# JuliaReinforcementLearning/ReinforcementLearning.jl

Measured on NVIDIA H100. Metric: env-steps/sec at 65536 CartPole envs (full PPO iteration: rollout T=32 + GAE + 4 epochs x 4 minibatches), higher is better.
Workload: dtype f32

## Files before the change

### reinforcementlearning.jl_b200/csrc/nn_tc.cu

```cuda
#include "nn.cuh"
#include "perm.cuh"
#include "policy.cuh"
#include "tc_fwd.cuh"
#include "tc_split.h"
#include "wgmma.cuh"

namespace {

using tcfwd::G_F;
using tcfwd::GW_S;
using tcfwd::WIMG_BYTES;
using tcfwd::split2;
using tcfwd::wimg_off;
constexpr int TM = tcfwd::TM;
constexpr int H = tcfwd::H;
constexpr float kScaleW = tcfwd::kScale;

constexpr int NT7 = 512;
constexpr int kMaxStage = 10;
constexpr int GF_T = 128;
constexpr int GS_T = 16 * GF_T;
constexpr int FIMG = 8 * GS_T;
constexpr float kScaleH = 64.0f, kScaleX = 64.0f;
constexpr int kNo = 2;

struct SmemBwd {
    static_assert(FIMG % 128 == 0 && WIMG_BYTES % 128 == 0 && (2 * GS_T) % 16 == 0, "operand images must stay 128-byte aligned");
    alignas(128) uint8_t FP_full[FIMG];
    alignas(128) uint8_t FP_lo[FIMG];
    alignas(128) uint8_t FH_lo[FIMG];
    alignas(128) uint8_t FH_full[FIMG];
    alignas(128) uint8_t FQ_full[FIMG];
    alignas(128) uint8_t FQ_lo[FIMG];
    alignas(128) uint8_t B1[WIMG_BYTES];
    alignas(128) uint8_t XT[2][2 * GS_T];
    alignas(128) uint8_t AH_full[FIMG];
    alignas(128) uint8_t AH_lo[FIMG];
    alignas(16) float D[TM * H];
    uint64_t H1pos[2][TM];
    float W1[kInMax * H];
    float b1[H], b2[H];
    float W3[H * kNo];
    float b3[kNo];
    float Zp[4 * kNo * TM];
    float Red[32];
    double RedD[16];
    float step_scale;
    alignas(8) uint64_t bar1;
    alignas(8) uint64_t bar3;
    alignas(8) uint64_t bar4;
    float AccW2[64 * 65 + 64];
    float AccD4[64 * 9];
};
__device__ __forceinline__ int d_off(int s, int col) { return s * H + ((((col >> 2) ^ (s & 15))) << 2) + (col & 3); }
__device__ __forceinline__ void d_ld16(const float* D, int s, int f0, float (&v)[16]) {
#pragma unroll
    for (int u = 0; u < 4; ++u) {
        const float4 q4 = *reinterpret_cast<const float4*>(D + d_off(s, f0 + 4 * u));
        v[4 * u] = q4.x; v[4 * u + 1] = q4.y; v[4 * u + 2] = q4.z; v[4 * u + 3] = q4.w;
    }
}
template <int TB>
__device__ __forceinline__ void gemm_ts3(float (&d)[32], const uint8_t* a_hi, const uint8_t* a_lo, int h, uint64_t dB, uint32_t b_step) {
    const uint64_t dA = wg::make_desc(wg::smem_u32(a_hi) + 8 * h * GF_T, GS_T, GF_T), dAl = wg::make_desc(wg::smem_u32(a_lo) + 8 * h * GF_T, GS_T, GF_T);
    wg::fence();
#pragma unroll
    for (int k = 0; k < 4; ++k) {
        const uint32_t aa = k * 2 * GS_T, bb = k * b_step;
        wg::mma_m64n64k16<0, TB>(d, wg::desc_add(dA, aa), wg::desc_add(dB, bb), k ? 1u : 0u);
        wg::mma_m64n64k16<0, TB>(d, wg::desc_add(dA, aa), wg::desc_add(dB, 8 * GW_S + bb), 1u);
        wg::mma_m64n64k16<0, TB>(d, wg::desc_add(dAl, aa), wg::desc_add(dB, bb), 1u);
    }
    wg::commit();
    wg::wait_all();
}
__device__ __forceinline__ uint32_t fimg_off(int f, int s) { return (uint32_t)((f >> 3) * GS_T + (s >> 3) * GF_T + (s & 7) * 16 + (f & 7) * 2); }
__device__ __forceinline__ void store16_feat(uint8_t* img, int f0, int s, const uint32_t (&v)[8]) {
    uint8_t* p = img + fimg_off(f0, s);
    *reinterpret_cast<uint4*>(p) = make_uint4(v[0], v[1], v[2], v[3]);
    *reinterpret_cast<uint4*>(p + GS_T) = make_uint4(v[4], v[5], v[6], v[7]);
}
using b200perm::perm_index;
using b200perm::perm_index_bits;

__device__ __forceinline__ float lane_transpose_reduce32(float (&v)[32], int lane) {
#pragma unroll
    for (int st = 0; st < 5; ++st) {
        const int half = 16 >> st, off = 16 >> st;
        const bool upper = (lane & off) != 0;
#pragma unroll
        for (int n = 0; n < half; ++n) {
            float send = upper ? v[n] : v[n + half];
            float keep = upper ? v[n + half] : v[n];
            v[n] = keep + __shfl_xor_sync(0xffffffffu, send, off);
        }
    }
    return v[0];
}

__device__ __forceinline__ void worker_sync() { asm volatile("bar.sync 1, 512;" ::: "memory"); }
__device__ __forceinline__ void group_sync(int q) { asm volatile("bar.sync %0, 128;" ::"r"(5 + q) : "memory"); }
__device__ __forceinline__ void ready_arrive(int id) { asm volatile("bar.arrive %0, 640;" ::"r"(id) : "memory"); }
__device__ __forceinline__ void ready_wait(int id) { asm volatile("bar.sync %0, 640;" ::"r"(id) : "memory"); }
#ifdef B200RL_K7_TIMING
__device__ unsigned long long g_k7_phase[40];
__device__ int g_k7_watch = 0;
#define K7_T(i) do { if (tid == (g_k7_watch & 0xFFFF) && (int)blockIdx.x == (g_k7_watch >> 16)) { long long now_ = clock64(); g_k7_phase[i] += (unsigned long long)(now_ - tprev_); tprev_ = now_; } } while (0)
#else
#define K7_T(i) do { } while (0)
#endif
constexpr int NT7_ALL = NT7 + 128;
constexpr int kRegsMma = 64, kRegsWorker = 104;
static_assert(128 * kRegsMma + NT7 * kRegsWorker <= NT7_ALL * 96, "setmaxnreg split must fit the CTA's register allocation");
constexpr int kBarRdyA = 2, kBarRdyB = 3;
constexpr int kBarMma = 4;
__device__ __forceinline__ void mma_sync() { asm volatile("bar.sync %0, 128;" ::"n"(kBarMma) : "memory"); }

template <int ACT>
__global__ void __launch_bounds__(NT7_ALL, 1)
ac_loss_grad_tc_kernel(MlpDesc actor, MlpDesc critic, const float* params , AcHyper hp, AcBatch b, float* partial,
                       float* __restrict__ loss_partial, int64_t np_total, float scale_base ,
                       OptStep st ,
                       int n_actor ) {
    extern __shared__ __align__(1024) unsigned char smem_raw[];
    SmemBwd& sm = *reinterpret_cast<SmemBwd*>(smem_raw);
    const int role = (int)blockIdx.x < n_actor ? 0 : 1;
    const int cta = role ? (int)blockIdx.x - n_actor : (int)blockIdx.x;
    const int nctas = role ? (int)gridDim.x - n_actor : n_actor;
    const int nrows = max(n_actor, (int)gridDim.x - n_actor);
    const float scale_p = scale_base * (role ? 4.0f : 64.0f);
    const MlpDesc d = role ? critic : actor;
    const int act = ACT >= 0 ? ACT : d.act;
    const bool relu = act == B200RL_ACT_RELU;
    const int64_t poff = role ? actor.nparams() : 0;
    const float* __restrict__ p = params + poff;
    const int tid = threadIdx.x, warp = tid >> 5, lane = tid & 31;
    const int q = warp & 3, c = (warp >> 2) & 3;
    const int s = 32 * q + lane;
    {
        const float* b1 = p + (int64_t)H * d.in;
        const float* W2 = b1 + H;
        const float* b2 = W2 + (int64_t)H * H;
        const float s1 = relu ? kScaleH : 1.0f;
        for (int k = tid; k < kInMax * H; k += NT7_ALL) sm.W1[k] = (k / H) < d.in ? p[k] * s1 : 0.f;
        for (int k = tid; k < H; k += NT7_ALL) { sm.b1[k] = b1[k] * s1; sm.b2[k] = b2[k]; }
        for (int k = tid; k < H * kNo; k += NT7_ALL) {
            int j = k / kNo, o = k % kNo;
            sm.W3[k] = o < d.nout ? p[head_w<false>(d, o, j)] : 0.f;
        }
        if (tid < kNo) sm.b3[tid] = tid < d.nout ? p[head_b<false>(d, tid)] : 0.f;
        tcfwd::fill_w2_image<NT7_ALL>(sm.B1, W2);
    }
    if (tid == 32) {
        wg::mbar_init(&sm.bar1, 128); wg::mbar_init(&sm.bar3, 128); wg::mbar_init(&sm.bar4, 128);
    }
    wg::fence_proxy_async();
    __syncthreads();
    const float inv_s1 = 1.0f / (kScaleH * kScaleW), inv_s3 = 1.0f / (scale_p * kScaleH), inv_sp = 1.0f / scale_p, inv_s4 = 1.0f / (scale_p * kScaleX);
    const int64_t ntiles = (b.B + TM - 1) / TM;

    if (warp >= NT7 / 32) {
        asm volatile("setmaxnreg.dec.sync.aligned.u32 %0;" ::"n"(kRegsMma));
        const int t = tid - NT7, row0 = 16 * (t >> 5) + ((t & 31) >> 2), col0 = 2 * (t & 3);
        const uint64_t dB1k = wg::make_desc(wg::smem_u32(sm.B1), G_F, GW_S);
        const uint64_t dB1t = wg::make_desc(wg::smem_u32(sm.B1), GW_S, G_F);
        float dacc[32];
        auto store_d = [&](int h) {
#pragma unroll
            for (int j = 0; j < 8; ++j)
#pragma unroll
                for (int hh = 0; hh < 2; ++hh)
                    *reinterpret_cast<float2*>(sm.D + d_off(64 * h + row0 + 8 * hh, 8 * j + col0)) = make_float2(dacc[4 * j + 2 * hh], dacc[4 * j + 2 * hh + 1]);
        };
        auto gemm1 = [&](int h) { gemm_ts3<0>(dacc, sm.AH_full, sm.AH_lo, h, dB1k, 2 * G_F); };
        auto gemm2 = [&](int h) { gemm_ts3<1>(dacc, sm.FP_full, sm.FP_lo, h, dB1t, 2 * GW_S); };
        auto store_dp1 = [&](int h, int pbuf) {
#pragma unroll
            for (int hh = 0; hh < 2; ++hh) {
                const int ss = 64 * h + row0 + 8 * hh;
                const uint64_t pos = relu ? sm.H1pos[pbuf][ss] >> col0 : 0u;
#pragma unroll
                for (int j = 0; j < 8; ++j) {
                    const uint32_t off = fimg_off(8 * j + col0, ss);
                    float v0 = dacc[4 * j + 2 * hh] * (1.0f / kScaleW), v1 = dacc[4 * j + 2 * hh + 1] * (1.0f / kScaleW);
                    if (relu) {
                        v0 = ((pos >> (8 * j)) & 1u) ? v0 : 0.f;
                        v1 = ((pos >> (8 * j + 1)) & 1u) ? v1 : 0.f;
                    } else {
                        const float inv_h = 1.0f / kScaleH;
                        const float2 hf = __half22float2(*reinterpret_cast<const __half2*>(sm.FH_full + off));
                        const float2 lf = __half22float2(*reinterpret_cast<const __half2*>(sm.FH_lo + off));
                        v0 *= dact_f(act, (hf.x + lf.x) * inv_h);
                        v1 *= dact_f(act, (hf.y + lf.y) * inv_h);
                    }
                    uint32_t hi, lo;
                    split2(v0, v1, hi, lo);
                    *reinterpret_cast<uint32_t*>(sm.FQ_full + off) = hi;
                    *reinterpret_cast<uint32_t*>(sm.FQ_lo + off) = lo;
                }
            }
        };
        auto gemm3 = [&](int buf) {
            const uint64_t dPh = wg::make_desc(wg::smem_u32(sm.FP_full), GF_T, GS_T), dPl = wg::make_desc(wg::smem_u32(sm.FP_lo), GF_T, GS_T);
            const uint64_t dHh = wg::make_desc(wg::smem_u32(sm.FH_full), GF_T, GS_T), dHl = wg::make_desc(wg::smem_u32(sm.FH_lo), GF_T, GS_T);
            wg::fence();
#pragma unroll
            for (int k = 0; k < 8; ++k) {
                const uint32_t a = k * 2 * GF_T;
                wg::mma_m64n64k16<1, 1>(dacc, wg::desc_add(dPh, a), wg::desc_add(dHh, a), k ? 1u : 0u);
                wg::mma_m64n64k16<1, 1>(dacc, wg::desc_add(dPl, a), wg::desc_add(dHh, a), 1u);
                wg::mma_m64n64k16<1, 1>(dacc, wg::desc_add(dPh, a), wg::desc_add(dHl, a), 1u);
            }
            wg::commit();
            wg::wait_all();
#pragma unroll
            for (int j = 0; j < 8; ++j)
#pragma unroll
                for (int hh = 0; hh < 2; ++hh)
#pragma unroll
                    for (int e = 0; e < 2; ++e) sm.AccW2[(row0 + 8 * hh) * 65 + 8 * j + col0 + e] += dacc[4 * j + 2 * hh + e];
            const uint64_t dX = wg::make_desc(wg::smem_u32(sm.XT[buf]), GF_T, GS_T);
            float d8[4] = {0.f, 0.f, 0.f, 0.f};
            wg::fence();
#pragma unroll
            for (int k = 0; k < 8; ++k) {
                const uint32_t a = k * 2 * GF_T;
                wg::mma_m64n8k16<1, 1>(d8, wg::desc_add(dPh, a), wg::desc_add(dX, a), k ? 1u : 0u);
                wg::mma_m64n8k16<1, 1>(d8, wg::desc_add(dPl, a), wg::desc_add(dX, a), 1u);
            }
            wg::commit();
            wg::wait_all();
            if (col0 == 4) {
                sm.AccW2[64 * 65 + row0] += d8[0];
                sm.AccW2[64 * 65 + row0 + 8] += d8[2];
            }
        };
        auto gemm4 = [&](int buf) {
            const uint64_t dQh = wg::make_desc(wg::smem_u32(sm.FQ_full), GF_T, GS_T), dQl = wg::make_desc(wg::smem_u32(sm.FQ_lo), GF_T, GS_T);
            const uint64_t dX = wg::make_desc(wg::smem_u32(sm.XT[buf]), GF_T, GS_T);
            float d4[4] = {0.f, 0.f, 0.f, 0.f};
            wg::fence();
#pragma unroll
            for (int k = 0; k < 8; ++k) {
                const uint32_t a = k * 2 * GF_T;
                wg::mma_m64n8k16<1, 1>(d4, wg::desc_add(dQh, a), wg::desc_add(dX, a), k ? 1u : 0u);
                wg::mma_m64n8k16<1, 1>(d4, wg::desc_add(dQh, a), wg::desc_add(dX, GS_T + a), 1u);
                wg::mma_m64n8k16<1, 1>(d4, wg::desc_add(dQl, a), wg::desc_add(dX, a), 1u);
            }
            wg::commit();
            wg::wait_all();
#pragma unroll
            for (int hh = 0; hh < 2; ++hh)
#pragma unroll
                for (int e = 0; e < 2; ++e)
                    if (col0 + e < 5) sm.AccD4[(row0 + 8 * hh) * 9 + col0 + e] += d4[2 * hh + e];
        };
        if (cta < ntiles) {
            ready_wait(kBarRdyB);
            for (int h = 0; h < 2; ++h) { gemm1(h); store_d(h); }
            wg::mbar_arrive(&sm.bar1);
        }
        int buf = 0;
        for (int64_t tile = cta; tile < ntiles; tile += nctas, buf ^= 1) {
            ready_wait(kBarRdyA);
            for (int h = 0; h < 2; ++h) { gemm2(h); store_dp1(h, buf); }
            wg::fence_proxy_async();
            if (tile + nctas < ntiles) {
                ready_wait(kBarRdyB);
                for (int h = 0; h < 2; ++h) { gemm1(h); store_d(h); }
                wg::mbar_arrive(&sm.bar1);
            }
            gemm3(buf);
            wg::mbar_arrive(&sm.bar3);
            mma_sync();
            gemm4(buf);
            wg::mbar_arrive(&sm.bar4);
        }
    } else {
    asm volatile("setmaxnreg.inc.sync.aligned.u32 %0;" ::"n"(kRegsWorker));
    float g3[2][16];
    float gb3a0 = 0.f, gb3a1 = 0.f;
#pragma unroll
    for (int k = 0; k < 16; ++k) { g3[0][k] = 0.f; g3[1][k] = 0.f; }
    float l0 = 0.f, l1 = 0.f;
    float mean = 0.f, inv_std = 1.f;
    if (hp.normalize_adv && b.norm2) { mean = b.norm2[0]; inv_std = b.norm2[1]; }
    uint32_t ph1 = 0, ph3 = 0, ph4 = 0;
    bool gemm4_pending = false;
    int xbuf = 0;
    int pbuf = 0;
#ifdef B200RL_K7_TIMING
    long long tprev_ = clock64();
#endif
    const int pbits = b200perm::perm_bits(b.perm_n);
    const uint32_t pkey = ac_perm_key(b);
    auto index_of = [&](int64_t t) -> int32_t {
        const int64_t j = t * TM + s;
        if (t >= ntiles || j >= b.B) return -1;
        return b.idx ? b.idx[j] : (int32_t)perm_index_bits((uint32_t)(b.perm_offset + j), b.perm_n, pkey, pbits);
    };
    auto request = [&](int32_t g, float (&x)[kInMax], float (&a)[4]) {
#pragma unroll
        for (int k = 0; k < kInMax; ++k) { x[k] = 0.f; a[k] = 0.f; }
        if (g < 0) return;
        if (b.rec) {
            const float4 v0 = b.rec[2 * (int64_t)g], v1 = b.rec[2 * (int64_t)g + 1];
            x[0] = v0.x; x[1] = v0.y; x[2] = v0.z; x[3] = v0.w;
            a[0] = v1.x; a[1] = v1.y; a[2] = v1.z; a[3] = v1.w;
        } else {
#pragma unroll
            for (int i = 0; i < kInMax; ++i)
                if (i < b.ns) x[i] = b.states[(int64_t)b.ns * g + i];
            a[0] = reinterpret_cast<const float*>(b.actions)[g];
            a[1] = b.logp_old ? b.logp_old[g] : 0.f;
            a[2] = b.adv[g];
            a[3] = b.ret[g];
        }
    };
    float pfx[kInMax] = {0.f, 0.f, 0.f, 0.f}, pfa[4] = {0.f, 0.f, 0.f, 0.f};
    float aux[4] = {0.f, 0.f, 0.f, 0.f};
    int32_t gi_next = -1;
    bool gemm3_pending = false;
    float* const out = partial + (int64_t)cta * np_total + poff;
    float* const gW1 = out;
    float* const gb1 = out + (int64_t)H * d.in;
    float* const gW2 = gb1 + H;
    float* const gb2 = gW2 + (int64_t)H * H;
    for (int k = tid; k < 64 * 65 + 64; k += NT7) sm.AccW2[k] = 0.f;
    for (int k = tid; k < 64 * 9; k += NT7) sm.AccD4[k] = 0.f;
    float xo[kInMax];
    auto publish = [&](int64_t t) {
#pragma unroll
        for (int i = 0; i < kInMax; ++i) xo[i] = pfx[i];
        aux[0] = pfa[0];
        aux[1] = role == 0 ? pfa[1] : 0.f;
        aux[2] = role == 0 ? (hp.normalize_adv ? (pfa[2] - mean) * inv_std : pfa[2]) : 0.f;
        aux[3] = role == 0 ? 0.f : pfa[3];
        if (c == 0) {
            uint32_t h01, l01, h23, l23;
            split2(xo[0] * kScaleX, xo[1] * kScaleX, h01, l01);
            split2(xo[2] * kScaleX, xo[3] * kScaleX, h23, l23);
            uint8_t* xt = sm.XT[xbuf] + fimg_off(0, s);
            *reinterpret_cast<uint4*>(xt) = make_uint4(h01, h23, 0x3C00u, 0u);
            *reinterpret_cast<uint4*>(xt + GS_T) = make_uint4(l01, l23, 0u, 0u);
        }
        K7_T(16);
        xbuf ^= 1;
        request(gi_next, pfx, pfa);
        gi_next = index_of(t + 2 * nctas);
        K7_T(17);
    };
    auto layer1 = [&]() {
        uint32_t pos = 0;
        uint32_t hi8[8], lo8[8];
#pragma unroll
        for (int ch = 0; ch < 4; ++ch) {
            const int f0 = 16 * c + 4 * ch;
            float4 bb = *reinterpret_cast<const float4*>(sm.b1 + f0);
            float h[4] = {bb.x, bb.y, bb.z, bb.w};
#pragma unroll
            for (int k = 0; k < kInMax; ++k) {
                float4 w = *reinterpret_cast<const float4*>(sm.W1 + k * H + f0);
                h[0] = fmaf(w.x, xo[k], h[0]); h[1] = fmaf(w.y, xo[k], h[1]); h[2] = fmaf(w.z, xo[k], h[2]); h[3] = fmaf(w.w, xo[k], h[3]);
            }
            if (relu) {
#pragma unroll
                for (int e = 0; e < 4; ++e) { pos |= (h[e] > 0.f ? 1u : 0u) << (4 * ch + e); h[e] = fmaxf(h[e], 0.f); }
            } else {
#pragma unroll
                for (int e = 0; e < 4; ++e) h[e] = act_f(act, h[e]) * kScaleH;
            }
            split2(h[0], h[1], hi8[2 * ch], lo8[2 * ch]);
            split2(h[2], h[3], hi8[2 * ch + 1], lo8[2 * ch + 1]);
        }
        if (relu) reinterpret_cast<uint16_t*>(&sm.H1pos[pbuf][s])[c] = (uint16_t)pos;
        pbuf ^= 1;
        store16_feat(sm.AH_full, 16 * c, s, hi8);
        store16_feat(sm.AH_lo, 16 * c, s, lo8);
    };
    if (cta < ntiles) {
        request(index_of(cta), pfx, pfa);
        gi_next = index_of(cta + nctas);
        publish(cta);
        layer1();
        wg::fence_proxy_async();
        ready_arrive(kBarRdyB);
    }
#ifdef B200RL_K7_TIMING
    tprev_ = clock64();
#endif
    for (int64_t tile = cta; tile < ntiles; tile += nctas) {
        const bool has_next = tile + nctas < ntiles;
        wg::mbar_wait(&sm.bar1, ph1);
        ph1 ^= 1u;
        K7_T(0);
        float h2[16];
        {
            float v[16];
            d_ld16(sm.D, s, 16 * c, v);
            float zp[kNo] = {0.f, 0.f};
#pragma unroll
            for (int k = 0; k < 16; ++k) {
                const int f = 16 * c + k;
                h2[k] = act_f(act, fmaf(v[k], inv_s1, sm.b2[f]));
                float2 w = *reinterpret_cast<const float2*>(sm.W3 + f * kNo);
                zp[0] = fmaf(w.x, h2[k], zp[0]); zp[1] = fmaf(w.y, h2[k], zp[1]);
            }
#pragma unroll
            for (int o = 0; o < kNo; ++o) sm.Zp[(c * kNo + o) * TM + s] = zp[o];
        }
        K7_T(1);
        group_sync(q);
        K7_T(2);
        {
            float z[kNo];
#pragma unroll
            for (int o = 0; o < kNo; ++o)
                z[o] = sm.b3[o] + ((sm.Zp[o * TM + s] + sm.Zp[(kNo + o) * TM + s]) + (sm.Zp[(2 * kNo + o) * TM + s] + sm.Zp[(3 * kNo + o) * TM + s]));
            const bool valid = (tile * TM + s) < b.B;
            const policy::LossOut<kNo> lo_ = policy::sample_loss(actor.heads2, actor.nout, role, hp, b.inv_B, z, aux[0], aux[1], aux[2], aux[3]);
            float dz[kNo];
#pragma unroll
            for (int o = 0; o < kNo; ++o) dz[o] = valid ? lo_.dz[o] : 0.f;
            if (c == 0 && valid) { l0 += lo_.l0; l1 += lo_.l1; gb3a0 += dz[0]; gb3a1 += dz[1]; }
            const float dzs0 = dz[0] * scale_p, dzs1 = dz[1] * scale_p;
            float dp[16];
#pragma unroll
            for (int k = 0; k < 16; ++k) {
                const int f = 16 * c + k;
                float2 w = *reinterpret_cast<const float2*>(sm.W3 + f * kNo);
                const float dh = fmaf(w.x, dzs0, w.y * dzs1);
                dp[k] = relu ? (h2[k] > 0.f ? dh : 0.f) : dh * (1.f - h2[k] * h2[k]);
                g3[0][k] = fmaf(dz[0], h2[k], g3[0][k]);
                g3[1][k] = fmaf(dz[1], h2[k], g3[1][k]);
            }
            uint32_t hi8[8], lo8[8];
#pragma unroll
            for (int m = 0; m < 8; ++m) split2(dp[2 * m], dp[2 * m + 1], hi8[m], lo8[m]);
            K7_T(3);
            if (gemm3_pending) {
                wg::mbar_wait(&sm.bar3, ph3);
                ph3 ^= 1u;
                gemm3_pending = false;
            }
            K7_T(4);
            store16_feat(sm.FP_full, 16 * c, s, hi8);
            store16_feat(sm.FP_lo, 16 * c, s, lo8);
            {
                const uint32_t off = fimg_off(16 * c, s);
                const uint4 h0 = *reinterpret_cast<const uint4*>(sm.AH_full + off), h1 = *reinterpret_cast<const uint4*>(sm.AH_full + off + GS_T);
                const uint4 l0 = *reinterpret_cast<const uint4*>(sm.AH_lo + off), l1 = *reinterpret_cast<const uint4*>(sm.AH_lo + off + GS_T);
                *reinterpret_cast<uint4*>(sm.FH_full + off) = h0; *reinterpret_cast<uint4*>(sm.FH_full + off + GS_T) = h1;
                *reinterpret_cast<uint4*>(sm.FH_lo + off) = l0; *reinterpret_cast<uint4*>(sm.FH_lo + off + GS_T) = l1;
            }
        }
        K7_T(5);
        wg::fence_proxy_async();
        if (gemm4_pending) {
            wg::mbar_wait(&sm.bar4, ph4);
            ph4 ^= 1u;
        }
        K7_T(6);
        ready_arrive(kBarRdyA);
        gemm3_pending = true;
        gemm4_pending = true;
        K7_T(7);
        if (has_next) {
            publish(tile + nctas);
            layer1();
            wg::fence_proxy_async();
            K7_T(8);
            ready_arrive(kBarRdyB);
            K7_T(9);
        }
#ifdef B200RL_K7_TIMING
        if (tid == (g_k7_watch & 0xFFFF) && (int)blockIdx.x == (g_k7_watch >> 16)) g_k7_phase[15] += 1;
#endif
    }
    if (gemm3_pending) wg::mbar_wait(&sm.bar3, ph3);
    if (gemm4_pending) wg::mbar_wait(&sm.bar4, ph4);
    worker_sync();
    for (int k = tid; k < H * H; k += NT7) gW2[k] = sm.AccW2[(k & 63) * 65 + (k >> 6)] * inv_s3;
    if (tid < H) {
        gb2[tid] = sm.AccW2[64 * 65 + tid] * inv_sp;
        gb1[tid] = sm.AccD4[tid * 9 + 4] * inv_sp;
        for (int i = 0; i < d.in; ++i) gW1[tid + H * i] = sm.AccD4[tid * 9 + i] * inv_s4;
    }
    if (cta >= (int)gridDim.x - nctas) {
        const int64_t ooff = role ? 0 : actor.nparams(), on = role ? actor.nparams() : critic.nparams();
        float* orow = partial + (int64_t)cta * np_total + ooff;
        for (int64_t kk = tid; kk < on; kk += NT7) orow[kk] = 0.f;
    }
    float* red = reinterpret_cast<float*>(sm.FP_full);
    static_assert(offsetof(SmemBwd, XT) - offsetof(SmemBwd, FP_full) >= (2 * TM * 65 + 2 * 8 * 64) * 4, "drain scratch");
    {
        constexpr int RS = 65;
        float* seg = red + 2 * TM * RS;
#pragma unroll
        for (int k = 0; k < 16; ++k) {
            red[0 * TM * RS + s * RS + 16 * c + k] = g3[0][k];
            red[1 * TM * RS + s * RS + 16 * c + k] = g3[1][k];
        }
        worker_sync();
        {
            const int col = tid & 63, g = tid >> 6;
#pragma unroll
            for (int m = 0; m < 2; ++m) {
                float a = 0.f;
#pragma unroll
                for (int ss = 0; ss < 16; ++ss) a += red[m * TM * RS + (16 * g + ss) * RS + col];
                seg[(m * 8 + g) * 64 + col] = a;
            }
        }
        worker_sync();
        if (tid < 2 * H) {
            const int m = tid >> 6, col = tid & 63;
            float a = 0.f;
#pragma unroll
            for (int g = 0; g < 8; ++g) a += seg[(m * 8 + g) * 64 + col];
            if (m < d.nout) out[head_w<false>(d, m, col)] = a;
        }
        worker_sync();
    }
    if (c == 0) { red[s] = gb3a0; red[TM + s] = gb3a1; }
    worker_sync();
    if (warp < d.nout) {
        float a = (red[warp * TM + lane] + red[warp * TM + 32 + lane]) + (red[warp * TM + 64 + lane] + red[warp * TM + 96 + lane]);
#pragma unroll
        for (int o = 16; o > 0; o >>= 1) a += __shfl_xor_sync(0xffffffffu, a, o);
        if (lane == 0) out[head_b<false>(d, warp)] = a;
    }
    float t0 = l0, t1 = l1;
#pragma unroll
    for (int o = 16; o > 0; o >>= 1) { t0 += __shfl_xor_sync(0xffffffffu, t0, o); t1 += __shfl_xor_sync(0xffffffffu, t1, o); }
    worker_sync();
    if (lane == 0) { sm.Red[warp] = t0; sm.Red[16 + warp] = t1; }
    worker_sync();
    if (tid == 0) {
        float a0 = 0.f, a1 = 0.f;
        for (int k = 0; k < 16; ++k) { a0 += sm.Red[k]; a1 += sm.Red[16 + k]; }
        float* lp = loss_partial + (int64_t)blockIdx.x * 4;
        lp[0] = role ? 0.f : a0; lp[1] = role ? 0.f : a1; lp[2] = role ? a0 : 0.f; lp[3] = 0.f;
    }
    if (blockIdx.x == 0)
        for (int k = tid; k < 4 * (2 * nrows - (int)gridDim.x); k += NT7) loss_partial[4 * (int64_t)gridDim.x + k] = 0.f;
    if (st.params) {
        const unsigned int G = gridDim.x;
        K7_T(24);
        worker_sync();
        K7_T(25);
        if (tid == 0) optim::grid_barrier(st.counters, G);
        worker_sync();
        K7_T(26);
        const int per = (int)((np_total + G - 1) / G);
        const int64_t k = (int64_t)blockIdx.x * per + tid;
        const bool mine = tid < per && k < np_total;
        const unsigned int seq = st.tab.nranks > 1 ? *st.seq_ptr + 1u : 0u;
        float* stage = reinterpret_cast<float*>(sm.FP_full);
        const int nstage = per * nrows;
        const int64_t k0 = (int64_t)blockIdx.x * per;
        {
            float t[kMaxStage];
#pragma unroll
            for (int j = 0; j < kMaxStage; ++j) {
                const int e = tid + j * NT7;
                const int row = e / per, col = e - row * per;
                t[j] = (e < nstage && k0 + col < np_total) ? __ldcg(partial + (int64_t)row * np_total + k0 + col) : 0.f;
            }
#pragma unroll
            for (int j = 0; j < kMaxStage; ++j) {
                const int e = tid + j * NT7;
                if (e < nstage) stage[e] = t[j];
            }
        }
        float* lstage = stage + nstage;
        if (blockIdx.x == 0) {
            float t[2];
#pragma unroll
            for (int j = 0; j < 2; ++j) t[j] = tid + j * NT7 < 4 * (int)G ? __ldcg(loss_partial + tid + j * NT7) : 0.f;
#pragma unroll
            for (int j = 0; j < 2; ++j) if (tid + j * NT7 < 4 * (int)G) lstage[tid + j * NT7] = t[j];
        }
        float m_k = 0.f, v_k = 0.f, p_k = 0.f;
        if (mine) { m_k = st.m[k]; v_k = st.v[k]; p_k = st.params[k]; }
        worker_sync();
        K7_T(27);
        float gk = 0.f;
        if (mine) {
            for (int c0 = 0; c0 < nrows; c0 += 8) {
                float t[8];
#pragma unroll
                for (int j = 0; j < 8; ++j) t[j] = c0 + j < nrows ? stage[(c0 + j) * per + tid] : 0.f;
#pragma unroll
                for (int j = 0; j < 8; ++j) if (c0 + j < nrows) gk += t[j];
            }
        }
        float lsum = 0.f;
        const bool loss_thread = blockIdx.x == 0 && tid < 4;
        if (loss_thread) {
            for (unsigned int c0 = 0; c0 < G; c0 += 8) {
                float t[8];
#pragma unroll
                for (int j = 0; j < 8; ++j) t[j] = c0 + j < G ? lstage[(c0 + j) * 4 + tid] : 0.f;
#pragma unroll
                for (int j = 0; j < 8; ++j) if (c0 + j < G) lsum += t[j];
            }
        }
        if (st.tab.nranks > 1) {
            const unsigned slot = seq & 1u;
            if (mine) p2p_push(st.tab, 0, slot, (size_t)k, __float_as_uint(gk), seq);
            if (loss_thread) p2p_push(st.tab, 0, slot, (size_t)np_total + tid, __float_as_uint(lsum), seq);
            if (mine) gk = p2p_sum_ranks(st.tab, 0, slot, (size_t)k, gk, seq);
            if (loss_thread) lsum = p2p_sum_ranks(st.tab, 0, slot, (size_t)np_total + tid, lsum, seq);
        }
        if (loss_thread) optim::publish_loss(st, tid, lsum);
        double sq = (double)gk * (double)gk;
#pragma unroll
        for (int o = 16; o > 0; o >>= 1) sq += __shfl_xor_sync(0xffffffffu, sq, o);
        if (lane == 0) sm.RedD[warp] = sq;
        worker_sync();
        K7_T(28);
        if (warp == 0) {
            if (lane == 0) {
                double t = 0.0;
                for (int w = 0; w < NT7 / 32; ++w) t += sm.RedD[w];
                st.cta_sumsq[blockIdx.x] = t;
                optim::grid_barrier(st.counters + 1, G);
            }
            __syncwarp();
            K7_T(29);
            double part[8];
#pragma unroll
            for (int j = 0; j < 8; ++j) part[j] = (unsigned)(lane + 32 * j) < G ? __ldcg(st.cta_sumsq + lane + 32 * j) : 0.0;
            double tot = 0.0;
#pragma unroll
            for (int j = 0; j < 8; ++j) tot += part[j];
#pragma unroll
            for (int o = 16; o > 0; o >>= 1) tot += __shfl_xor_sync(0xffffffffu, tot, o);
            if (lane == 0) {
                const float gn = (float)sqrt(tot);
                sm.step_scale = optim::clip_scale(gn, st.max_norm);
                if (blockIdx.x == 0) optim::publish_gnorm(st, gn);
            }
        }
        worker_sync();
        K7_T(30);
        const float bt1 = st.beta_t[0], bt2 = st.beta_t[1];
        if (mine) {
            gk *= sm.step_scale;
            st.grad[k] = gk;
            const optim::AdamOut a = optim::adam_update(gk, m_k, v_k, p_k, st.lr, st.b1, st.b2, st.eps, bt1, bt2);
            st.m[k] = a.m; st.v[k] = a.v; st.params[k] = a.p;
        }
        worker_sync();
        if (tid == 0) optim::close_step<3>(st, bt1, bt2, st.tab.nranks > 1, seq);
        K7_T(31);
    }
    }
    __syncthreads();
}

}

int nn_tc_actor_ctas(int grid, const MlpDesc& actor, const AcHyper& hp, int64_t ntiles) {
    static int forced = -2;
    if (forced == -2) { const char* e = getenv("B200RL_K7_ACTOR_CTAS"); forced = e ? atoi(e) : -1; }
    if (forced > 0 && forced < grid) return forced;
    (void)hp;
    return b200rl_tc_actor_ctas(grid, actor.heads2 != 0, ntiles);
}
int nn_tc_partial_rows(int grid, const MlpDesc& actor, const AcHyper& hp, int64_t B) {
    const int na = nn_tc_actor_ctas(grid, actor, hp, (B + TM - 1) / TM);
    return na > grid - na ? na : grid - na;
}
bool nn_tc_bwd_supported(const MlpDesc& actor, const MlpDesc& critic) {
    return actor.H == 64 && critic.H == 64 && actor.in <= kInMax && actor.nout <= 2 && critic.nout == 1;
}
bool nn_tc_step_fits(b200rl_ctx* ctx, int grid, const MlpDesc& actor, const AcHyper& hp, int64_t B, int64_t np) {
    const int64_t per = (np + grid - 1) / grid;
    return grid <= ctx->sm_count && grid <= 256 && per <= NT7 && per * nn_tc_partial_rows(grid, actor, hp, B) <= kMaxStage * NT7 &&
           4 * grid <= 2 * NT7;
}
int nn_tc_ac_loss_grad(b200rl_ctx* ctx, int grid, const MlpDesc& actor, const MlpDesc& critic, const float* params, const AcHyper& hp,
                       const AcBatch& b, float* partial, float* loss_partial, int64_t np, const OptStep* step) {
    const OptStep st = step ? *step : OptStep{};
    const int n_actor = nn_tc_actor_ctas(grid, actor, hp, (b.B + TM - 1) / TM);
    size_t smem = sizeof(SmemBwd) + 128;
    static unsigned long long attr_devices = 0;
    if (first_use_on_device(attr_devices, ctx->device)) {
        CUDA_TRY(cudaFuncSetAttribute(ac_loss_grad_tc_kernel<B200RL_ACT_RELU>, cudaFuncAttributeMaxDynamicSharedMemorySize, (int)smem));
        CUDA_TRY(cudaFuncSetAttribute(ac_loss_grad_tc_kernel<B200RL_ACT_TANH>, cudaFuncAttributeMaxDynamicSharedMemorySize, (int)smem));
        CUDA_TRY(cudaFuncSetAttribute(ac_loss_grad_tc_kernel<-1>, cudaFuncAttributeMaxDynamicSharedMemorySize, (int)smem));
    }
    const float scale_base = exp2f(floorf(log2f(1.0f / b.inv_B)));
    if (actor.act == critic.act && actor.act == B200RL_ACT_RELU)
        ac_loss_grad_tc_kernel<B200RL_ACT_RELU><<<grid, NT7_ALL, smem, ctx->stream>>>(actor, critic, params, hp, b, partial, loss_partial, np, scale_base, st, n_actor);
    else if (actor.act == critic.act && actor.act == B200RL_ACT_TANH)
        ac_loss_grad_tc_kernel<B200RL_ACT_TANH><<<grid, NT7_ALL, smem, ctx->stream>>>(actor, critic, params, hp, b, partial, loss_partial, np, scale_base, st, n_actor);
    else
        ac_loss_grad_tc_kernel<-1><<<grid, NT7_ALL, smem, ctx->stream>>>(actor, critic, params, hp, b, partial, loss_partial, np, scale_base, st, n_actor);
    LAUNCH_CHECK(ctx);
    return B200RL_OK;
}

#ifdef B200RL_K7_TIMING
extern "C" int b200rl_debug_k7_watch(int tid) {
    cudaDeviceSynchronize();
    return cudaMemcpyToSymbol(g_k7_watch, &tid, sizeof tid) == cudaSuccess ? 0 : -1;
}
extern "C" int b200rl_debug_k7_phases(unsigned long long* out16, int reset) {
    cudaDeviceSynchronize();
    if (cudaMemcpyFromSymbol(out16, g_k7_phase, sizeof(unsigned long long) * 40) != cudaSuccess) return -1;
    if (reset) { unsigned long long z[24] = {0}; cudaMemcpyToSymbol(g_k7_phase, z, sizeof z); }
    return 0;
}
#endif
```

Measured before the change: 308.8 million.

## Specialize ReLU backward: split per-row loss, index, and X-image work across worker groups

```diff
diff --git a/reinforcementlearning.jl_b200/csrc/nn_tc.cu b/reinforcementlearning.jl_b200/csrc/nn_tc.cu
--- a/reinforcementlearning.jl_b200/csrc/nn_tc.cu
+++ b/reinforcementlearning.jl_b200/csrc/nn_tc.cu
@@ -51,8 +51,16 @@
     alignas(8) uint64_t bar4;
     float AccW2[64 * 65 + 64];
     float AccD4[64 * 9];
+    float DZ[kNo * TM];
+    int32_t GI[2][TM];
 };
+__device__ __forceinline__ uint8_t* h1_hi(SmemBwd& sm, int k) { return k ? sm.FH_full : sm.AH_full; }
+__device__ __forceinline__ uint8_t* h1_lo(SmemBwd& sm, int k) { return k ? sm.FH_lo : sm.AH_lo; }
 __device__ __forceinline__ int d_off(int s, int col) { return s * H + ((((col >> 2) ^ (s & 15))) << 2) + (col & 3); }
+__device__ __forceinline__ void d_st16(float* D, int s, int f0, const float (&v)[16]) {
+#pragma unroll
+    for (int u = 0; u < 4; ++u) *reinterpret_cast<float4*>(D + d_off(s, f0 + 4 * u)) = make_float4(v[4 * u], v[4 * u + 1], v[4 * u + 2], v[4 * u + 3]);
+}
 __device__ __forceinline__ void d_ld16(const float* D, int s, int f0, float (&v)[16]) {
 #pragma unroll
     for (int u = 0; u < 4; ++u) {
@@ -114,6 +122,7 @@
 static_assert(128 * kRegsMma + NT7 * kRegsWorker <= NT7_ALL * 96, "setmaxnreg split must fit the CTA's register allocation");
 constexpr int kBarRdyA = 2, kBarRdyB = 3;
 constexpr int kBarMma = 4;
+constexpr int kLossC = 0, kIdxC = 1, kXtC = 2;
 __device__ __forceinline__ void mma_sync() { asm volatile("bar.sync %0, 128;" ::"n"(kBarMma) : "memory"); }
 
 template <int ACT>
@@ -132,6 +141,7 @@
     const MlpDesc d = role ? critic : actor;
     const int act = ACT >= 0 ? ACT : d.act;
     const bool relu = act == B200RL_ACT_RELU;
+    constexpr bool lean = ACT == B200RL_ACT_RELU;
     const int64_t poff = role ? actor.nparams() : 0;
     const float* __restrict__ p = params + poff;
     const int tid = threadIdx.x, warp = tid >> 5, lane = tid & 31;
@@ -172,7 +182,7 @@
                 for (int hh = 0; hh < 2; ++hh)
                     *reinterpret_cast<float2*>(sm.D + d_off(64 * h + row0 + 8 * hh, 8 * j + col0)) = make_float2(dacc[4 * j + 2 * hh], dacc[4 * j + 2 * hh + 1]);
         };
-        auto gemm1 = [&](int h) { gemm_ts3<0>(dacc, sm.AH_full, sm.AH_lo, h, dB1k, 2 * G_F); };
+        auto gemm1 = [&](int h, int abuf) { gemm_ts3<0>(dacc, h1_hi(sm, abuf), h1_lo(sm, abuf), h, dB1k, 2 * G_F); };
         auto gemm2 = [&](int h) { gemm_ts3<1>(dacc, sm.FP_full, sm.FP_lo, h, dB1t, 2 * GW_S); };
         auto store_dp1 = [&](int h, int pbuf) {
 #pragma unroll
@@ -188,8 +198,8 @@
                         v1 = ((pos >> (8 * j + 1)) & 1u) ? v1 : 0.f;
                     } else {
                         const float inv_h = 1.0f / kScaleH;
-                        const float2 hf = __half22float2(*reinterpret_cast<const __half2*>(sm.FH_full + off));
-                        const float2 lf = __half22float2(*reinterpret_cast<const __half2*>(sm.FH_lo + off));
+                        const float2 hf = __half22float2(*reinterpret_cast<const __half2*>(h1_hi(sm, lean ? pbuf : 1) + off));
+                        const float2 lf = __half22float2(*reinterpret_cast<const __half2*>(h1_lo(sm, lean ? pbuf : 1) + off));
                         v0 *= dact_f(act, (hf.x + lf.x) * inv_h);
                         v1 *= dact_f(act, (hf.y + lf.y) * inv_h);
                     }
@@ -202,7 +212,8 @@
         };
         auto gemm3 = [&](int buf) {
             const uint64_t dPh = wg::make_desc(wg::smem_u32(sm.FP_full), GF_T, GS_T), dPl = wg::make_desc(wg::smem_u32(sm.FP_lo), GF_T, GS_T);
-            const uint64_t dHh = wg::make_desc(wg::smem_u32(sm.FH_full), GF_T, GS_T), dHl = wg::make_desc(wg::smem_u32(sm.FH_lo), GF_T, GS_T);
+            const int hb = lean ? buf : 1;
+            const uint64_t dHh = wg::make_desc(wg::smem_u32(h1_hi(sm, hb)), GF_T, GS_T), dHl = wg::make_desc(wg::smem_u32(h1_lo(sm, hb)), GF_T, GS_T);
             wg::fence();
 #pragma unroll
             for (int k = 0; k < 8; ++k) {
@@ -257,7 +268,7 @@
         };
         if (cta < ntiles) {
             ready_wait(kBarRdyB);
-            for (int h = 0; h < 2; ++h) { gemm1(h); store_d(h); }
+            for (int h = 0; h < 2; ++h) { gemm1(h, 0); store_d(h); }
             wg::mbar_arrive(&sm.bar1);
         }
         int buf = 0;
@@ -267,7 +278,7 @@
             wg::fence_proxy_async();
             if (tile + nctas < ntiles) {
                 ready_wait(kBarRdyB);
-                for (int h = 0; h < 2; ++h) { gemm1(h); store_d(h); }
+                for (int h = 0; h < 2; ++h) { gemm1(h, lean ? buf ^ 1 : 0); store_d(h); }
                 wg::mbar_arrive(&sm.bar1);
             }
             gemm3(buf);
@@ -289,6 +300,7 @@
     bool gemm4_pending = false;
     int xbuf = 0;
     int pbuf = 0;
+    int gpar = 0;
 #ifdef B200RL_K7_TIMING
     long long tprev_ = clock64();
 #endif
@@ -304,17 +316,22 @@
         for (int k = 0; k < kInMax; ++k) { x[k] = 0.f; a[k] = 0.f; }
         if (g < 0) return;
         if (b.rec) {
-            const float4 v0 = b.rec[2 * (int64_t)g], v1 = b.rec[2 * (int64_t)g + 1];
+            const float4 v0 = b.rec[2 * (int64_t)g];
             x[0] = v0.x; x[1] = v0.y; x[2] = v0.z; x[3] = v0.w;
-            a[0] = v1.x; a[1] = v1.y; a[2] = v1.z; a[3] = v1.w;
+            if (c == kLossC || !lean) {
+                const float4 v1 = b.rec[2 * (int64_t)g + 1];
+                a[0] = v1.x; a[1] = v1.y; a[2] = v1.z; a[3] = v1.w;
+            }
         } else {
 #pragma unroll
             for (int i = 0; i < kInMax; ++i)
                 if (i < b.ns) x[i] = b.states[(int64_t)b.ns * g + i];
-            a[0] = reinterpret_cast<const float*>(b.actions)[g];
-            a[1] = b.logp_old ? b.logp_old[g] : 0.f;
-            a[2] = b.adv[g];
-            a[3] = b.ret[g];
+            if (c == kLossC || !lean) {
+                a[0] = reinterpret_cast<const float*>(b.actions)[g];
+                a[1] = b.logp_old ? b.logp_old[g] : 0.f;
+                a[2] = b.adv[g];
+                a[3] = b.ret[g];
+            }
         }
     };
     float pfx[kInMax] = {0.f, 0.f, 0.f, 0.f}, pfa[4] = {0.f, 0.f, 0.f, 0.f};
@@ -332,11 +349,13 @@
     auto publish = [&](int64_t t) {
 #pragma unroll
         for (int i = 0; i < kInMax; ++i) xo[i] = pfx[i];
-        aux[0] = pfa[0];
-        aux[1] = role == 0 ? pfa[1] : 0.f;
-        aux[2] = role == 0 ? (hp.normalize_adv ? (pfa[2] - mean) * inv_std : pfa[2]) : 0.f;
-        aux[3] = role == 0 ? 0.f : pfa[3];
-        if (c == 0) {
+        if (c == kLossC || !lean) {
+            aux[0] = pfa[0];
+            aux[1] = role == 0 ? pfa[1] : 0.f;
+            aux[2] = role == 0 ? (hp.normalize_adv ? (pfa[2] - mean) * inv_std : pfa[2]) : 0.f;
+            aux[3] = role == 0 ? 0.f : pfa[3];
+        }
+        if (c == (lean ? kXtC : 0)) {
             uint32_t h01, l01, h23, l23;
             split2(xo[0] * kScaleX, xo[1] * kScaleX, h01, l01);
             split2(xo[2] * kScaleX, xo[3] * kScaleX, h23, l23);
@@ -347,7 +366,9 @@
         K7_T(16);
         xbuf ^= 1;
         request(gi_next, pfx, pfa);
-        gi_next = index_of(t + 2 * nctas);
+        if (b.idx || !lean) gi_next = index_of(t + 2 * nctas);
+        else if (c == kIdxC) sm.GI[gpar][s] = index_of(t + 2 * nctas);
+        gpar ^= 1;
         K7_T(17);
     };
     auto layer1 = [&]() {
@@ -374,9 +395,9 @@
             split2(h[2], h[3], hi8[2 * ch + 1], lo8[2 * ch + 1]);
         }
         if (relu) reinterpret_cast<uint16_t*>(&sm.H1pos[pbuf][s])[c] = (uint16_t)pos;
+        store16_feat(h1_hi(sm, lean ? pbuf : 0), 16 * c, s, hi8);
+        store16_feat(h1_lo(sm, lean ? pbuf : 0), 16 * c, s, lo8);
         pbuf ^= 1;
-        store16_feat(sm.AH_full, 16 * c, s, hi8);
-        store16_feat(sm.AH_lo, 16 * c, s, lo8);
     };
     if (cta < ntiles) {
         request(index_of(cta), pfx, pfa);
@@ -412,17 +433,30 @@
         K7_T(1);
         group_sync(q);
         K7_T(2);
-        {
+        float dz[kNo];
+        if (c == kLossC || !lean) {
+            if (lean) d_st16(sm.D, s, 16 * c, h2);
             float z[kNo];
 #pragma unroll
             for (int o = 0; o < kNo; ++o)
                 z[o] = sm.b3[o] + ((sm.Zp[o * TM + s] + sm.Zp[(kNo + o) * TM + s]) + (sm.Zp[(2 * kNo + o) * TM + s] + sm.Zp[(3 * kNo + o) * TM + s]));
             const bool valid = (tile * TM + s) < b.B;
             const policy::LossOut<kNo> lo_ = policy::sample_loss(actor.heads2, actor.nout, role, hp, b.inv_B, z, aux[0], aux[1], aux[2], aux[3]);
-            float dz[kNo];
 #pragma unroll
             for (int o = 0; o < kNo; ++o) dz[o] = valid ? lo_.dz[o] : 0.f;
-            if (c == 0 && valid) { l0 += lo_.l0; l1 += lo_.l1; gb3a0 += dz[0]; gb3a1 += dz[1]; }
+            if (c == kLossC && valid) { l0 += lo_.l0; l1 += lo_.l1; gb3a0 += dz[0]; gb3a1 += dz[1]; }
+            if (lean) {
+#pragma unroll
+                for (int o = 0; o < kNo; ++o) sm.DZ[o * TM + s] = dz[o];
+                group_sync(q);
+                d_ld16(sm.D, s, 16 * c, h2);
+            }
+        } else {
+            group_sync(q);
+#pragma unroll
+            for (int o = 0; o < kNo; ++o) dz[o] = sm.DZ[o * TM + s];
+        }
+        {
             const float dzs0 = dz[0] * scale_p, dzs1 = dz[1] * scale_p;
             float dp[16];
 #pragma unroll
@@ -446,7 +480,7 @@
             K7_T(4);
             store16_feat(sm.FP_full, 16 * c, s, hi8);
             store16_feat(sm.FP_lo, 16 * c, s, lo8);
-            {
+            if (!lean) {
                 const uint32_t off = fimg_off(16 * c, s);
                 const uint4 h0 = *reinterpret_cast<const uint4*>(sm.AH_full + off), h1 = *reinterpret_cast<const uint4*>(sm.AH_full + off + GS_T);
                 const uint4 l0 = *reinterpret_cast<const uint4*>(sm.AH_lo + off), l1 = *reinterpret_cast<const uint4*>(sm.AH_lo + off + GS_T);
@@ -466,6 +500,7 @@
         gemm4_pending = true;
         K7_T(7);
         if (has_next) {
+            if (lean && !b.idx) gi_next = sm.GI[gpar ^ 1][s];
             publish(tile + nctas);
             layer1();
             wg::fence_proxy_async();
@@ -522,7 +557,7 @@
         }
         worker_sync();
     }
-    if (c == 0) { red[s] = gb3a0; red[TM + s] = gb3a1; }
+    if (c == kLossC) { red[s] = gb3a0; red[TM + s] = gb3a1; }
     worker_sync();
     if (warp < d.nout) {
         float a = (red[warp * TM + lane] + red[warp * TM + 32 + lane]) + (red[warp * TM + 64 + lane] + red[warp * TM + 96 + lane]);
```

Result: faster. 315.3 million, median of 6 (+2.1%).
